# mpieva/network-aware-bwa

Measured on AMD Instinct MI355X. Metric: aligned reads/s to GRCh38 (100 bp SE), FM-index search (bwa_cal_sa_reg_gap), bit-exact vs CPU, higher is better.
Workload: dtype u32

## Files before the change

network-aware-bwa_amd/csrc/fm_index.hip:

```cpp
#include "nabwa_dev.hpp"
#include "launchers.hpp"

__device__ __forceinline__ uint32_t ref_base(const uint32_t *w, uint32_t j)
{
	const uint32_t *p = w + (size_t)(j >> 7) * 12 + 4;
	return p[(j & 127u) >> 4] >> ((~j & 15u) << 1) & 3u;
}

__global__ __launch_bounds__(256) void repack_kernel(const uint32_t *__restrict__ w, uint32_t seq_len,
													 uint32_t n_buckets, uint4 *__restrict__ out)
{
	const uint32_t b = blockIdx.x * 256u + threadIdx.x;
	if (b >= n_buckets) return;
	const uint32_t j0 = b * NABWA_INTV;
	uint32_t cnt[4] = {0, 0, 0, 0};
	if (j0 <= seq_len) {
		const uint32_t blk = j0 >> 7;
		const uint32_t *p = w + (size_t)blk * 12;
		cnt[0] = p[0]; cnt[1] = p[1]; cnt[2] = p[2]; cnt[3] = p[3];
		for (uint32_t j = blk << 7; j < j0; ++j) ++cnt[ref_base(w, j)];
	}
	uint64_t lo[3] = {0, 0, 0}, hi[3] = {0, 0, 0};
	for (uint32_t g = 0; g < 3; ++g) {
		for (uint32_t q = 0; q < 4; ++q) {
// ... 50 lines not shown
	k /= intv;
	out[idx] = steps + (k ? sa[k] : 0xffffffffu);
}

extern "C" void nabwa_launch_sa_lookup(const DevBwt *B, int n, const uint8_t *which, const uint32_t *k, uint32_t *out,
									   hipStream_t s)
{
	if (n <= 0) return;
	hipLaunchKernelGGL(sa_lookup_kernel, dim3((n + 255) / 256), dim3(256), 0, s, B[0], B[1], n, which, k, out);
}

__global__ __launch_bounds__(256) void occ4_kernel(DevBwt B, int n, const uint32_t *__restrict__ k, uint32_t *__restrict__ out)
{
	const int idx = blockIdx.x * 256 + threadIdx.x;
	if (idx >= n) return;
	const Occ4 o = nabwa_occ4(B, k[idx]);
	out[4 * idx] = o.c[0]; out[4 * idx + 1] = o.c[1]; out[4 * idx + 2] = o.c[2]; out[4 * idx + 3] = o.c[3];
}

extern "C" void nabwa_launch_occ4(const DevBwt *B, int n, const uint32_t *k, uint32_t *out, hipStream_t s)
{
	if (n <= 0) return;
	hipLaunchKernelGGL(occ4_kernel, dim3((n + 255) / 256), dim3(256), 0, s, *B, n, k, out);
}

__global__ __launch_bounds__(256) void kmer_level_kernel(DevBwt B, const uint2 *__restrict__ prev, uint2 *__restrict__ cur, uint64_t n_par)
{
	const uint64_t idx = (uint64_t)blockIdx.x * 256u + threadIdx.x;
	if (idx >= n_par) return;
	const uint2 par = prev ? prev[idx] : make_uint2(0u, B.seq_len);
	uint2 out[4];
#pragma unroll
	for (int c = 0; c < 4; ++c) out[c] = make_uint2(1u, 0u);
	if (par.x <= par.y) {
		Occ4 ck, cl;
		nabwa_occ4_pair(B, par.x - 1u, par.y, ck, cl);
#pragma unroll
		for (int c = 0; c < 4; ++c) {
			const uint32_t k = B.L2[c] + ck.c[c] + 1u, l = B.L2[c] + cl.c[c];
			if (k <= l) out[c] = make_uint2(k, l);
		}
	}
	uint4 *const dst = (uint4*)(cur + 4 * idx);
	dst[0] = make_uint4(out[0].x, out[0].y, out[1].x, out[1].y);
	dst[1] = make_uint4(out[2].x, out[2].y, out[3].x, out[3].y);
}

extern "C" void nabwa_launch_kmer_level(const DevBwt *B, const uint2 *prev, uint2 *cur, uint64_t n_cur, hipStream_t s)
{
	const uint64_t n_par = n_cur / 4;
	hipLaunchKernelGGL(kmer_level_kernel, dim3((unsigned int)((n_par + 255) / 256)), dim3(256), 0, s, *B, prev, cur, n_par);
}

__global__ __launch_bounds__(256) void sa_fill_kernel(DevBwt B, uint32_t *__restrict__ sa_full, uint32_t *__restrict__ isa,
												  uint8_t *__restrict__ text_bytes)
{
	const uint32_t j = blockIdx.x * 256u + threadIdx.x;
	if (j >= B.n_sa) return;
	uint32_t row = j * B.sa_intv, v = j ? B.sa[j] : B.seq_len;
	sa_full[row] = j ? v : 0xffffffffu;
	isa[v] = row;
	for (;;) {
		if (row == B.primary) break;
		const uint32_t kp = row - (row > B.primary ? 1u : 0u);
		const uint32_t b = kp / NABWA_INTV, r = kp - b * NABWA_INTV;
		const uint4 *p = B.bk + (size_t)b * 4;
		const uint4 q0 = p[0], q1 = p[1], q2 = p[2], q3 = p[3];
		const uint32_t c = nabwa_base_at(q1, q2, q3, r);
		const Occ4 o = nabwa_count4(q0, q1, q2, q3, r);
		v -= 1u;
		text_bytes[v] = (uint8_t)c;
		row = B.L2[c] + o.c[c];
		if (row % B.sa_intv == 0u) break;
		sa_full[row] = v; isa[v] = row;
	}
}

__global__ __launch_bounds__(256) void text_pack_kernel(const uint8_t *__restrict__ bytes, uint32_t n, uint32_t n_words, uint32_t *__restrict__ out)
{
	const uint32_t w = blockIdx.x * 256u + threadIdx.x;
	if (w >= n_words) return;
	uint32_t x = 0;
	for (uint32_t t = 0; t < 16u; ++t) { const uint64_t j = (uint64_t)w * 16u + t; if (j < n) x |= (uint32_t)(bytes[j] & 3u) << (2u * t); }
	out[w] = x;
}

extern "C" void nabwa_launch_sa_fill(const DevBwt *B, uint32_t *sa_full, uint32_t *isa, uint8_t *text_bytes, hipStream_t s)
{
	hipLaunchKernelGGL(sa_fill_kernel, dim3((B->n_sa + 255) / 256), dim3(256), 0, s, *B, sa_full, isa, text_bytes);
}
extern "C" void nabwa_launch_text_pack(const uint8_t *bytes, uint32_t n, uint32_t n_words, uint32_t *out, hipStream_t s)
{
	hipLaunchKernelGGL(text_pack_kernel, dim3((n_words + 255) / 256), dim3(256), 0, s, bytes, n, n_words, out);
}
```

network-aware-bwa_amd/csrc/fm_search.hip:

```cpp
#include "nabwa_dev.hpp"
#include "fm_search.hpp"
#include "launchers.hpp"

#define STATE_M 0
#define STATE_I 1
#define STATE_D 2
#define STATE_GROUP 3
#define GRP_EXT 0x100u
#define TXM 0xfffffffeu
#define KEYM 0xffffffffu
#define LVO(t_) ((size_t)((((uint64_t)1 << (2 * (t_))) - 4ull) / 3ull))
#ifndef NABWA_W_WAVES
#define NABWA_W_WAVES 5
#endif
#ifndef NABWA_WORK_CHUNK
#define NABWA_WORK_CHUNK 64u
#endif
#ifndef NABWA_RUN_MAX
#define NABWA_RUN_MAX 4
#endif

__device__ __forceinline__ uint32_t byte_of(uint64_t lo, uint64_t hi, uint32_t idx)
{
	asm volatile("" : "+v"(lo), "+v"(hi));
	const uint64_t h = (idx & 8u) ? hi : lo;
	return (uint32_t)(h >> ((idx & 7u) << 3)) & 0xffu;
}
#define WIN_SET(lo_, hi_, a_, b_, c_, d_) do { lo_ = (uint64_t)(b_) << 32 | (a_); hi_ = (uint64_t)(d_) << 32 | (c_); } while (0)

__device__ __forceinline__ void set_word(uint4 &q, uint32_t c, uint32_t v)
{
	q.x = c == 0 ? v : q.x; q.y = c == 1 ? v : q.y; q.z = c == 2 ? v : q.z; q.w = c == 3 ? v : q.w;
}

extern __shared__ uint16_t s_head[];

#ifndef NABWA_MIN_WAVES
#define NABWA_MIN_WAVES 4
#endif

template <bool COUNT>
__global__ __launch_bounds__(NABWA_SEARCH_BLOCK, NABWA_W_WAVES) void fm_width_kernel(const SearchParams P)
{
	const uint32_t lane = threadIdx.x & 63u;
	bool run = false, done = false;
	unsigned int w_next = 0, w_end = 0;
	uint32_t rid = 0, x = 0; int len = 0, phase = 0, wi = 0, n = 0, sbase = 0, nN = 0;
	uint32_t sq_off = 0;
#define WREC (P.wdata + (size_t)rid * P.wstride)
#define BX(f_) (x ? P.bwt[1].f_ : P.bwt[0].f_)
	bool tmode = false; uint32_t tp = 0, twtag = 0xffffffffu; uint2 twin = make_uint2(0u, 0u);
	const bool text_ok = (P.text_mode & 1) && P.bwt[0].sa_full && P.bwt[1].sa_full;
	uint32_t kk = 0, ll = 0, pw = 0; int bid = 0;
	uint32_t wkey = 0xffffffffu; bool tok = false; int tbase = 0;
	const int KT = (int)P.bwt[0].kmer_T, LW = (int)P.bwt[0].kmer_LW;
	auto rekey = [&](int from) {
		tok = false; tbase = from;
		if (!KT || !P.rd_pack || from + 4 >= n) return;
		const int PW = P.pack_stride / 2;
		const uint32_t *const pk = P.rd_pack + (size_t)rid * P.pack_stride + x * PW;
		if (pk[PW - 1]) return;
		const int q = sbase + from;
		const uint32_t w0 = pk[q >> 4], w1 = pk[(q >> 4) + 1], sh = ((uint32_t)q & 15u) << 1;
		const uint32_t k16 = sh ? (w0 << sh) | (w1 >> (32u - sh)) : w0;
		wkey = k16 >> (2 * (16 - KT)); tok = true;
	};
	uint4 wacc = make_uint4(0, 0, 0, 0); uint64_t blo = 0, bhi = 0, slo = 0, shi = 0; int stag = -1;
	unsigned long long touches = 0;

	for (;;) {
		unsigned long long need = __ballot(!run && !done);
		if (P.w_sync && __ballot(run) != 0ull) need = 0ull;
		if (need) {
			if (w_next == w_end) {
				unsigned int base = 0;
				if (lane == 0) base = atomicAdd(P.work_counter + WC_WIDTH, (unsigned int)NABWA_WORK_CHUNK);
				w_next = __builtin_amdgcn_readfirstlane(base); w_end = w_next + NABWA_WORK_CHUNK;
			}
			const unsigned int rank = (unsigned int)__popcll(need & ((1ull << lane) - 1ull)), avail = w_end - w_next;
			const unsigned int base = w_next;
			w_next += min((unsigned int)__popcll(need), avail);
			if (!run && !done && rank < avail) {
				const unsigned int idx = base + rank;
				if (idx < 2u * (unsigned int)P.n) {
					rid = P.ids ? (uint32_t)P.ids[idx >> 1] : idx >> 1; x = idx & 1u;
					const int64_t o = P.poff[rid];
					len = P.rd_len[rid];
					sq_off = (uint32_t)o;
					nN = 0; stag = -1;
					if (P.w_skip_clean && P.n_aln[rid] == 0) {  }
					else if (len > 0) {
						run = true; phase = 0; wi = 0; n = len; sbase = 0; tmode = false;
						if (KT) { wkey = P.rd_key[6 * (size_t)rid + 2 + x]; tok = wkey != 0xffffffffu; }
						tbase = 0;
						kk = 0; ll = BX(seq_len); bid = 0; pw = 0; blo = bhi = 0;
					} else { if (x == 0u) P.rd_nN[rid] = 0; if (P.rd_cls) P.rd_cls[2 * (size_t)rid + x] = 0; }
				} else done = true;
			}
		}
		if (__ballot(!done) == 0ull) break;
		auto out_pos = [&](int p, bool last) {
			uint8_t *const rec = WREC;
			if (last) ++bid;
			const uint32_t wv = last ? 0u : ll - kk + 1u;
			const uint32_t bv = (uint32_t)(bid > 127 ? 127 : bid) | ((p > 0 && wv == pw) ? 128u : 0u);
			set_word(wacc, (uint32_t)p & 3u, wv);
			{ const uint64_t sh = (uint64_t)bv << (((uint32_t)p & 7u) << 3); if (p & 8) bhi |= sh; else blo |= sh; }
			pw = wv;
			if (phase == 0 && ((p & 3) == 3 || last)) *(uint4*)((uint32_t*)rec + x * P.WL + (p & ~3)) = wacc;
			if ((p & 15) == 15 || last) {
				*(uint4*)(rec + (phase ? P.woff_sbid + x * P.SLB : P.woff_bid + x * P.WLB) + (p & ~15)) =
					make_uint4((uint32_t)blo, (uint32_t)(blo >> 32), (uint32_t)bhi, (uint32_t)(bhi >> 32));
				blo = bhi = 0;
			}
		};
		bool bulk = run && phase == 0 && tmode && (wi & 15) == 0 && wi + 16 < n && tp >= 16u && pw == 1u;
		if (bulk) {
			if ((wi >> 4) != stag) { const uint4 q = *(const uint4*)((x ? P.rseq : P.seq) + sq_off + wi); WIN_SET(slo, shi, q.x, q.y, q.z, q.w); stag = wi >> 4; }
			const uint32_t w0 = (tp - 16u) >> 4;
			const uint32_t *const txt = BX(text);
			const uint32_t t0 = txt[w0], t1 = txt[w0 + 1u];
			auto squeeze = [](uint64_t v) -> uint32_t {
				uint64_t y = v & 0x0303030303030303ull;
				y = (y | y >> 6) & 0x000F000F000F000Full; y = (y | y >> 12) & 0x000000FF000000FFull; y = (y | y >> 24) & 0xFFFFull;
				return (uint32_t)y;
			};
			const bool clean = ((slo | shi) & 0xFCFCFCFCFCFCFCFCull) == 0ull;
			const uint32_t rd = squeeze(slo) | squeeze(shi) << 16;
			const uint32_t tx = (uint32_t)(((uint64_t)t1 << 32 | t0) >> (((tp - 16u) & 15u) << 1));
			uint32_t rv = __brev(tx); rv = (rv >> 1 & 0x55555555u) | (rv & 0x55555555u) << 1;
			bulk = clean && rv == rd;
			if (bulk) {
				uint8_t *const rec = WREC;
				uint32_t *const wp = (uint32_t*)rec + x * P.WL + wi;
#pragma unroll
				for (int u = 0; u < 4; ++u) *(uint4*)(wp + 4 * u) = make_uint4(1u, 1u, 1u, 1u);
				const uint32_t b4 = ((uint32_t)(bid > 127 ? 127 : bid) | 128u) * 0x01010101u;
				*(uint4*)(rec + P.woff_bid + x * P.WLB + wi) = make_uint4(b4, b4, b4, b4);
				tp -= 16u; wi += 16;
			}
		}
		if (bulk) {  }
		else if (run && tok && wi - tbase + 4 <= LW && wi + 4 < n) {
			uint2 tv[4];
			const uint2 *const lo = BX(kmer_lo);
#pragma unroll
			for (int u = 0; u < 4; ++u) {
				const int t = wi - tbase + u + 1;
				tv[u] = (lo + (size_t)((((uint64_t)1 << (2 * t)) - 4ull) / 3ull))[wkey >> (2 * (KT - t))];
			}
#pragma unroll
			for (int u = 0; u < 4; ++u) {
				kk = tv[u].x; ll = tv[u].y;
				const bool dead = kk > ll;
				if (dead) { kk = 0; ll = BX(seq_len); ++bid; }
				out_pos(wi, false);
				++wi;
				if (dead) { rekey(wi); break; }
			}
		} else if (run) {
			const int pos = sbase + wi;
			if ((pos >> 4) != stag) { const uint4 q = *(const uint4*)((x ? P.rseq : P.seq) + sq_off + (pos & ~15)); WIN_SET(slo, shi, q.x, q.y, q.z, q.w); stag = pos >> 4; }
			const int cc = (int)byte_of(slo, shi, (uint32_t)pos & 15u);
			uint4 qa[4], qb[4]; uint32_t rk = 0, rl = 0, sav = 0; bool kval = false, two = false;
#pragma unroll
			for (int u = 0; u < 4; ++u) { qa[u] = make_uint4(0, 0, 0, 0); qb[u] = make_uint4(0, 0, 0, 0); }
			const bool q = cc < 4 && !tmode;
			if (q) {
				const uint32_t primary = BX(primary), kq = kk - 1u, lq = ll;
				const uint32_t kp = kq - (kq >= primary ? 1u : 0u), lp = lq - (lq >= primary ? 1u : 0u);
				const uint32_t bl = lp / NABWA_INTV; rl = lp - bl * NABWA_INTV;
				kval = kq != 0xffffffffu;
				const uint32_t bkk = kval ? kp / NABWA_INTV : bl; rk = kp - bkk * NABWA_INTV;
				two = bkk != bl;
				const uint4 *const bkt = BX(bk);
				const uint4 *pl = bkt + (size_t)bl * 4, *pk = bkt + (size_t)bkk * 4;
#pragma unroll
				for (int u = 0; u < 4; ++u) qa[u] = pl[u];
				if (two) {
#pragma unroll
					for (int u = 0; u < 4; ++u) qb[u] = pk[u];
				}
				if (COUNT) touches += ref_touches(x ? P.bwt[1] : P.bwt[0], kq, lq, false);
				if (text_ok && kk == ll) sav = BX(sa_full)[kk];
			}
			if (tmode && tp > 0u && ((tp - 1u) >> 5) != twtag) {
				twtag = (tp - 1u) >> 5;
				twin = *(const uint2*)(BX(text) + 2 * (size_t)twtag);
			}
			if (tmode) {
				bool ok = cc < 4 && tp > 0u;
				if (ok) {
					const uint32_t t = tp - 1u, wd = (t & 16u) ? twin.y : twin.x;
					ok = (wd >> ((t & 15u) << 1) & 3u) == (uint32_t)cc;
					if (ok) tp = t;
				}
				if (cc > 3 && x == 0u && phase == 0) ++nN;
				if (!ok) { tmode = false; kk = 0; ll = BX(seq_len); ++bid; rekey(wi + 1); }
			} else {
				const bool was_one = text_ok && cc < 4 && kk == ll;
				if (cc < 4) {
					Occ4 ck, cl;
// ... 733 lines not shown
```

network-aware-bwa_amd/csrc/fm_search.hpp:

```cpp
#pragma once
#include <stdint.h>
#include "nabwa_dev.hpp"
#include "search_slots.hpp"

#define NABWA_SEARCH_BLOCK 256
#define NABWA_ST_OK        0
#define NABWA_ST_OVERFLOW  1
#define NABWA_ST_WIDE      2
#define NABWA_ST_POOL      3
#define NABWA_ST_HITCAP    4
#define NABWA_ST_GROWN     5

struct SearchParams {
	DevBwt bwt[2];
	const uint8_t *seq, *rseq;
	const int64_t *poff;
	const int32_t *rd_len;
	const uint8_t *rd_maxdiff, *rd_maxgapo;
	const int32_t *ids;
	const int32_t *res_slot;
	int n;
	int s_mm, s_gapo, s_gape, mode, indel_end_skip, max_del_occ, max_entries, max_gape, max_seed_diff, seed_len, max_top2;
	uint8_t *wdata;
	size_t wstride;
	uint32_t woff_bid, woff_sbid;
	uint32_t WL, WLB, SLB;
	int text_mode;
	const uint32_t *rd_key;
	uint8_t *rd_nN;
	uint8_t *scratch;
	size_t lane_stride;
	uint32_t cap, NS;
	int32_t *n_aln, *max_ent;
	uint8_t *status;
	uint4 *aln;
	int aln_cap;
	unsigned int *work_counter;
	uint32_t trip_budget;
	uint32_t trip_budget_hard;
	int sync_refill;
	const uint32_t *rd_pack; int pack_stride;
	int w_sync;
	int w_skip_clean;
	uint8_t *rd_cls;
	const unsigned int *n_sync;
	unsigned long long *touch_counter;
	const uint32_t *ixtab;
	int sure0;
	unsigned long long *s0_stats;
};

#define NABWA_IXTAB_STRIDE 24
#define NABWA_IXTAB_WORDS  48
#define IX_BK 0
#define IX_KMER 2
#define IX_KMER_LO 4
#define IX_TEXT 6
#define IX_ISA 8
#define IX_SA_FULL 10
#define IX_PRIMARY 12
#define IX_SEQ_LEN 13
#define IX_L2 13
static inline void nabwa_ixtab_fill(uint32_t *tab, const DevBwt *bwt )
{
	for (int q = 0; q < 2; ++q) {
		uint32_t *o = tab + NABWA_IXTAB_STRIDE * q;
		const uint64_t p[6] = { (uint64_t)(uintptr_t)bwt[q].bk, (uint64_t)(uintptr_t)bwt[q].kmer, (uint64_t)(uintptr_t)bwt[q].kmer_lo,
								(uint64_t)(uintptr_t)bwt[q].text, (uint64_t)(uintptr_t)bwt[q].isa, (uint64_t)(uintptr_t)bwt[q].sa_full };
		for (int f = 0; f < 6; ++f) { o[2 * f] = (uint32_t)p[f]; o[2 * f + 1] = (uint32_t)(p[f] >> 32); }
		o[IX_PRIMARY] = bwt[q].primary; o[IX_SEQ_LEN] = bwt[q].seq_len; o[IX_L2 + 1] = bwt[q].L2[1]; o[IX_L2 + 2] = bwt[q].L2[2]; o[IX_L2 + 3] = bwt[q].L2[3];
		for (int f = 17; f < NABWA_IXTAB_STRIDE; ++f) o[f] = 0;
	}
}
```

network-aware-bwa_amd/csrc/launchers.hpp:

```cpp
#pragma once
#include <hip/hip_runtime.h>
#include "fm_deep.hpp"

extern "C" {
void nabwa_launch_repack(const uint32_t *w, uint32_t seq_len, uint32_t n_buckets, uint4 *out, hipStream_t s);
void nabwa_launch_kmer_level(const DevBwt *B, const uint2 *prev, uint2 *cur, uint64_t n_cur, hipStream_t s);
void nabwa_launch_sa_fill(const DevBwt *B, uint32_t *sa_full, uint32_t *isa, uint8_t *text_bytes, hipStream_t s);
void nabwa_launch_text_pack(const uint8_t *bytes, uint32_t n, uint32_t n_words, uint32_t *out, hipStream_t s);
void nabwa_launch_sa_lookup(const DevBwt *B, int n, const uint8_t *which, const uint32_t *k, uint32_t *out, hipStream_t s);
void nabwa_launch_occ4(const DevBwt *B, int n, const uint32_t *k, uint32_t *out, hipStream_t s);
void nabwa_launch_fm_search(const SearchParams *P, int n_blocks, hipStream_t s);
void nabwa_launch_fm_width(const SearchParams *P, int n_blocks, hipStream_t s);
int nabwa_width_occupancy(void);
int nabwa_search_occupancy(int ns);
void nabwa_launch_checksum(int n, const int32_t *map, const uint32_t *cent, const uint8_t *arena, const int32_t *n_aln, const uint4 *aln, int aln_cap, const uint8_t *status,
						   const int32_t *wide_idx, const uint4 *aln2, int aln_cap2, const uint4 *const *grown,
						   unsigned long long *sum, unsigned long long *rows, hipStream_t s);
void nabwa_launch_collect(int n, const uint8_t *status, int32_t *ids, unsigned int *count, int which, hipStream_t s);
void nabwa_launch_collect_keyed(int n, const uint8_t *status, int32_t *ids, unsigned int *count, int which,
								const uint8_t *cls, const uint8_t *md, int max_key, const int32_t *n_aln, int aln_cap, hipStream_t s);
void nabwa_launch_assign_slots(int n2, const int32_t *ids, int32_t *wide_idx, hipStream_t s);
void nabwa_launch_scatter_grown(int n2, const int32_t *ids, const int32_t *n_aln3, const int32_t *max_ent3, const uint8_t *status3,
								 int32_t *n_aln, int32_t *max_ent, uint8_t *status, int32_t *wide_idx, const uint4 *block, size_t cap3,
								 const uint4 **grown, int slot0, hipStream_t s);
void nabwa_launch_scatter_wide(int n2, const int32_t *ids, const int32_t *n_aln2, const int32_t *max_ent2,
							   const uint8_t *status2, int32_t *n_aln, int32_t *max_ent, uint8_t *status,
							   int32_t *wide_idx, hipStream_t s);
void nabwa_launch_gather(int n, const int32_t *map, const uint32_t *cent, const uint8_t *arena, const int32_t *n_aln, const uint32_t *row_off, const uint4 *aln, int aln_cap,
						 const uint8_t *status, const int32_t *wide_idx, const uint4 *aln2, int aln_cap2,
						 const uint4 *const *grown, uint4 *out, hipStream_t s);
void nabwa_launch_partition(int n, const uint8_t *cls, int32_t *ids, unsigned int *cnt, hipStream_t s);
void nabwa_launch_padded_len(int n, const int64_t *off, int64_t *plen, hipStream_t s);
void nabwa_launch_pad_reads(int n, const uint8_t *seq, const uint8_t *rseq, const int64_t *off, const int64_t *poff,
							uint8_t *pseq, uint8_t *prseq, int32_t *rd_len, uint32_t *rd_key, int T, int seed_len, uint32_t *rd_pack, int pack_stride,
							const uint8_t *md_tab, const uint8_t *mg_tab, uint8_t *rd_md, uint8_t *rd_mg, hipStream_t s);
void nabwa_launch_dedup_hash(int n, const uint8_t *seq, const uint8_t *rseq, const int64_t *off, uint64_t mask, uint64_t *keys, uint32_t *ids, hipStream_t s);
void nabwa_launch_dedup_heads(int n, const uint64_t *keys, uint32_t *head, hipStream_t s);
void nabwa_launch_dedup_verify(int n, const uint8_t *seq, const uint8_t *rseq, const int64_t *off, const uint32_t *ids, const uint32_t *head,
							   int32_t *rep, uint32_t *flag, unsigned int *n_coll, hipStream_t s);
void nabwa_launch_dedup_map(int n, const int32_t *rep, const uint32_t *inner, const int64_t *off, int32_t *map, int64_t *clen, unsigned int *stat, hipStream_t s);
void nabwa_launch_dedup_compact(int n, const uint8_t *seq, const uint8_t *rseq, const int64_t *off, const int32_t *rep, const uint32_t *inner,
								const int64_t *coff, uint8_t *cseq, uint8_t *crseq, hipStream_t s);
void nabwa_launch_dedup_expand(int n, const int32_t *map, const int32_t *n_aln, const int32_t *max_ent, const uint32_t *cent, const uint8_t *arena,
							   int32_t *n_aln_out, int32_t *max_ent_out, hipStream_t s);
void nabwa_launch_dcache_lookup(int n, const uint8_t *seq, const uint8_t *rseq, const int64_t *off, const uint64_t *hash, const uint8_t *md_tab, const uint8_t *mg_tab,
								const unsigned long long *slots, uint32_t n_slots, uint64_t mask, const uint8_t *arena, uint32_t *found, uint32_t *flag, hipStream_t s);
void nabwa_launch_dcache_map(int n, const uint32_t *found, const uint32_t *inner, const int64_t *off, int32_t *rep, int32_t *newidx, int64_t *clen, uint32_t *cent,
							 unsigned int *stat, hipStream_t s);
void nabwa_launch_dcache_remap(int n, const int32_t *old, const int32_t *newidx, int32_t *map, hipStream_t s);
void nabwa_launch_dcache_insert(int n, const uint8_t *seq, const uint8_t *rseq, const int64_t *poff, const int32_t *len, const uint8_t *rd_md, const uint8_t *rd_mg,
								const uint8_t *status, const int32_t *n_aln, const int32_t *max_ent, const uint4 *aln, int aln_cap, const int32_t *wide_idx,
								const uint4 *aln2, int aln_cap2, const uint4 *const *grown, int row_cap, uint64_t mask,
								unsigned long long *slots, uint32_t n_slots, uint8_t *arena, uint64_t arena_bytes, unsigned long long *ctr, hipStream_t s);
void nabwa_launch_fm_deep(const DeepParams *P, int n_waves, hipStream_t s);
int nabwa_deep_occupancy(int ns, int lds_rd);
void nabwa_launch_bgzf_deflate(const uint8_t *in, int64_t n, int n_slices, uint8_t *stage, uint32_t *sizes, hipStream_t s);
void nabwa_launch_bgzf_deflate_dyn(const uint8_t *in, int64_t n, int n_slices, uint8_t *stage, uint32_t *sizes, hipStream_t s);
void nabwa_launch_bgzf_pack(const uint8_t *stage, const uint32_t *sizes, int n_slices, uint8_t *packed, int64_t *total, hipStream_t s);
struct BgzfInBlk;
// ... 12 lines not shown
```

network-aware-bwa_amd/csrc/nabwa_batch.hip:

```cpp
#include <hip/hip_runtime.h>
#include <hipcub/hipcub.hpp>
#include <stdio.h>
#include <stdlib.h>
#include <string.h>
#include <memory>
#include <mutex>
#include <vector>
#include "../../include/nabwa.h"
#include "nabwa_batch.hpp"
#include "dedup_cache_body.hpp"
#include "host_util.hpp"

static void layout(SearchParams &P, uint32_t cap, int max_len, int seed_len, uint32_t NS)
{
	P.WL = align_up((uint32_t)max_len + 1, 16);
	P.WLB = P.WL + 16;
	P.SLB = align_up((uint32_t)(max_len > seed_len ? seed_len : 0) + 1, 16) + 16;
	P.woff_bid = 2 * P.WL * 4;
	P.woff_sbid = P.woff_bid + 2 * P.WLB;
	P.wstride = align_up(P.woff_sbid + 2 * P.SLB, 64);
	P.cap = cap; P.NS = NS;
	P.lane_stride = align_up((size_t)cap * 16, 64);
}

// ... 223 lines not shown
	if ((uint64_t)pnb >= (1ull << 32)) return nabwa_fail(NABWA_EINVAL, "batch holds 4 Gi padded bases or more: split it (lane state keeps a 32-bit read offset)");
	auto read_buffers = [&](int n) -> int {
		HIP_CHECK(b->d_seq.get(ix, pnb)); HIP_CHECK(b->d_rseq.get(ix, pnb));
		HIP_CHECK(b->d_poff.get(ix, (size_t)(n + 1) * 8)); HIP_CHECK(b->d_len.get(ix, (size_t)(n ? n : 1) * 4));
		HIP_CHECK(b->d_md.get(ix, n ? n : 1)); HIP_CHECK(b->d_mg.get(ix, n ? n : 1)); HIP_CHECK(b->d_key.get(ix, (size_t)(n ? n : 1) * 24));
		b->pack_stride = 2 * ((max_len + 15) / 16 + 2);
		HIP_CHECK(b->d_pack.get(ix, (size_t)(n ? n : 1) * b->pack_stride * 4));
		HIP_CHECK(b->d_cls.get(ix, (size_t)(n ? n : 1) * 2)); HIP_CHECK(b->d_perm.get(ix, (size_t)(n ? n : 1) * 4)); HIP_CHECK(b->d_ncls.get(ix, NCLS_WORDS * sizeof(unsigned int)));
		return NABWA_OK;
	};
	const bool dedup = dedup_bits >= 0 && n_given > 0;
	if (!dedup) if (int r = read_buffers(n_given)) return r;
	if (n_given == 0) { HIP_CHECK(hipMemset(b->d_poff, 0, 8)); return NABWA_OK; }
	PoolBuf<uint8_t> raw_s, raw_r, d_tab; PoolBuf<int64_t> raw_off, plen; PoolBuf<void> d_tmp; size_t tmp_bytes = 0;
	StreamDrain drain{ b->stream };
	HIP_CHECK(raw_s.get(ix, nb)); HIP_CHECK(raw_r.get(ix, nb)); HIP_CHECK(raw_off.get(ix, (size_t)(n_given + 1) * 8));
	const UploadJob jobs[3] = { { raw_s, seq, (size_t)off[n_given] }, { raw_r, rseq, (size_t)off[n_given] }, { raw_off, off, (size_t)(n_given + 1) * 8 } };
	const double tu0 = now_s();
	HIP_CHECK(staged_upload(ix, jobs, 3));
	if (timing) fprintf(stderr, "[nabwa] upload of %.2f GB: %.3f s (%.3f s into batch_create)\n", 2e-9 * (double)off[n_given], now_s() - tu0, tu0 - tc0);
	if (dedup) {
		if (int r = dedup_reads(b, dedup_bits, raw_s, raw_r, raw_off, nb, timing)) return r;
		if (b->cache) if (int r = cache_lookup(b, s, raw_s, raw_r, raw_off, nb, timing)) return r;
		if (int r = read_buffers(b->n)) return r;
	}
	const int n = b->n;
	HIP_CHECK(plen.get(ix, (size_t)(n + 1) * 8));
	nabwa_launch_padded_len(n, raw_off, plen, b->stream);
	HIP_CHECK(hipcub::DeviceScan::ExclusiveSum(nullptr, tmp_bytes, plen.p, b->d_poff.p, n + 1, b->stream));
	HIP_CHECK(d_tmp.get(ix, tmp_bytes ? tmp_bytes : 16));
	HIP_CHECK(hipcub::DeviceScan::ExclusiveSum(d_tmp.p, tmp_bytes, plen.p, b->d_poff.p, n + 1, b->stream));
	HIP_CHECK(d_tab.get(ix, 2 * (size_t)(max_len + 1)));
	HIP_CHECK(hipMemcpyAsync(d_tab, s.md_tab.data(), max_len + 1, hipMemcpyHostToDevice, b->stream));
	HIP_CHECK(hipMemcpyAsync(d_tab + max_len + 1, s.mg_tab.data(), max_len + 1, hipMemcpyHostToDevice, b->stream));
	nabwa_launch_pad_reads(n, raw_s, raw_r, raw_off, b->d_poff, b->d_seq, b->d_rseq, b->d_len, b->d_key,
						   ix->bwt[0].kmer_T == ix->bwt[1].kmer_T ? (int)ix->bwt[0].kmer_T : 0, b->opt.seed_len, b->d_pack, b->pack_stride,
						   d_tab, d_tab + max_len + 1, b->d_md, b->d_mg, b->stream);
	HIP_CHECK(hipStreamSynchronize(b->stream));
	if (timing) fprintf(stderr, "[nabwa] re-layout kernel done %.3f s into batch_create\n", now_s() - tc0);
	HIP_CHECK(raw_s.release()); HIP_CHECK(raw_r.release()); HIP_CHECK(raw_off.release());
	HIP_CHECK(plen.release()); HIP_CHECK(d_tmp.release()); HIP_CHECK(d_tab.release());
	return NABWA_OK;
}

static int working_buffers(nabwa_batch *b, const BatchShape &s)
{
	nabwa_index *ix = b->ix;
	const nabwa_gap_opt_t *opt = &b->opt;
	const int n = b->n, max_len = s.max_len;
	SearchParams &P = b->P;
	memset(&P, 0, sizeof(P));
	P.bwt[0] = ix->bwt[0]; P.bwt[1] = ix->bwt[1];
	{
		uint32_t tab[NABWA_IXTAB_WORDS];
		nabwa_ixtab_fill(tab, ix->bwt);
		HIP_CHECK(b->d_ixtab.get(ix, sizeof tab));
		HIP_CHECK(hipMemcpy(b->d_ixtab, tab, sizeof tab, hipMemcpyHostToDevice));
		P.ixtab = b->d_ixtab;
	}
	P.seq = b->d_seq; P.rseq = b->d_rseq; P.poff = b->d_poff; P.rd_len = b->d_len; P.rd_maxdiff = b->d_md; P.rd_maxgapo = b->d_mg; P.rd_key = b->d_key; P.rd_pack = b->d_pack; P.pack_stride = b->pack_stride;
	P.text_mode = env_int("NABWA_TEXT_KERNELS", 7);
	if (ix->bwt[0].kmer_T != ix->bwt[1].kmer_T) P.bwt[0].kmer_T = P.bwt[1].kmer_T = 0;
	P.ids = 0; P.n = n;
	P.s_mm = opt->s_mm; P.s_gapo = opt->s_gapo; P.s_gape = opt->s_gape; P.mode = opt->mode;
	P.indel_end_skip = opt->indel_end_skip; P.max_del_occ = opt->max_del_occ; P.max_entries = opt->max_entries;
	P.max_gape = opt->max_gape; P.max_seed_diff = opt->max_seed_diff; P.seed_len = opt->seed_len; P.max_top2 = opt->max_top2;
	int cap1 = env_int("NABWA_CAP1", 4096);
	if (cap1 < 16) cap1 = 16;
	if (cap1 > 65534) cap1 = 65534;
	layout(P, (uint32_t)cap1, max_len, opt->seed_len, s.deep_only ? 1u : s.NS1);
	P.aln_cap = env_int("NABWA_ALNCAP1", 16);
	P.sync_refill = env_int("NABWA_SYNC_REFILL", 0);
	P.trip_budget = (uint32_t)env_int("NABWA_TRIP_BUDGET", max_len > opt->seed_len ? 2000 : 300);
	P.trip_budget_hard = (uint32_t)env_int("NABWA_TRIP_BUDGET_HARD", max_len > opt->seed_len ? 200 : (int)P.trip_budget);
	if (getenv("NABWA_TRIP_BUDGET") && !getenv("NABWA_TRIP_BUDGET_HARD")) P.trip_budget_hard = P.trip_budget;
	b->class_sort = env_int("NABWA_CLASS_SORT", 1);
	P.sure0 = env_int("NABWA_SURE0", 3);
	if (P.sure0 < 0) P.sure0 = 0;
	if (P.sure0 > 3) P.sure0 = 3;
	if (env_int("NABWA_SURE0_STATS", 0)) {
		HIP_CHECK(b->d_s0stats.get(ix, S0S_WORDS * sizeof(unsigned long long)));
		HIP_CHECK(hipMemset(b->d_s0stats, 0, S0S_WORDS * sizeof(unsigned long long)));
		P.s0_stats = b->d_s0stats;
	}
	{
		P.w_sync = (n > 0 && s.min_len == max_len) ? env_int("NABWA_W_SYNC", 1) : 0;
	}
	if (P.aln_cap < 1) P.aln_cap = 1;

	hipDeviceProp_t prop;
	HIP_CHECK(hipGetDeviceProperties(&prop, ix->device));
	int occ = nabwa_search_occupancy(s.deep_only ? 1 : (int)s.NS1);
	if (occ < 1) occ = 1;
	const int occ_env = env_int("NABWA_BLOCKS_PER_CU", 0);
	if (occ_env > 0) occ = occ_env;
	long blocks = (long)prop.multiProcessorCount * occ;
	const long need = ((long)n + NABWA_SEARCH_BLOCK - 1) / NABWA_SEARCH_BLOCK;
	if (blocks > need) blocks = need;
	if (blocks < 1) blocks = 1;
	b->n_blocks = (int)blocks;
	if (getenv("NABWA_TIMING")) fprintf(stderr, "[nabwa] search kernel: %u score levels, %d blocks per CU (LDS %zu B per block), %ld blocks\n", s.NS1, occ,
										(size_t)s.NS1 * NABWA_SEARCH_BLOCK * 2 + NABWA_SEARCH_BLOCK * 80, blocks);
	HIP_CHECK(b->d_scratch.get(ix, (size_t)blocks * NABWA_SEARCH_BLOCK * P.lane_stride));
	int occw = nabwa_width_occupancy(); if (occw < 1) occw = 1;
	long blocks_w = (long)prop.multiProcessorCount * occw;
	if (blocks_w > 2 * need) blocks_w = 2 * need;
	if (blocks_w < 1) blocks_w = 1;
	b->n_blocks_w = (int)blocks_w;
	HIP_CHECK(b->d_wdata.get(ix, (size_t)(n ? n : 1) * P.wstride));
	HIP_CHECK(b->d_nN.get(ix, n ? n : 1));
	P.wdata = b->d_wdata; P.rd_nN = b->d_nN;
	const size_t n1 = n ? n : 1;
	HIP_CHECK(b->d_naln.get(ix, n1 * 4)); HIP_CHECK(b->d_maxent.get(ix, n1 * 4)); HIP_CHECK(b->d_wide_idx.get(ix, n1 * 4));
	HIP_CHECK(b->d_status.get(ix, n1)); HIP_CHECK(b->d_aln.get(ix, n1 * (size_t)P.aln_cap * 16));
// ... 379 lines not shown
```

network-aware-bwa_amd/csrc/nabwa_index.hip:

```cpp
#include <hip/hip_runtime.h>
#include <stdio.h>
#include <stdlib.h>
#include <string.h>
#include <memory>
#include <string>
#include <vector>
#include "../../include/nabwa.h"
#include "launchers.hpp"
#include "dedup_cache_body.hpp"
#include "nabwa_internal.hpp"
#include "dev_pool.hpp"
#include "finish_gpu.hpp"

static int build_one(nabwa_index *ix, int t_, const uint32_t *words, uint64_t n_words, bool on_device,
					 const uint32_t *sa_words, uint64_t n_sa_words)
{
	uint32_t hdr[5];
	if (n_words < 5) return nabwa_fail(NABWA_EIO, "bwt array too short");
	if (on_device) HIP_CHECK(hipMemcpy(hdr, words, 20, hipMemcpyDeviceToHost)); else memcpy(hdr, words, 20);
	DevBwt &B = ix->bwt[t_];
	memset(&B, 0, sizeof(B));
	B.primary = hdr[0]; B.L2[0] = 0; B.L2[1] = hdr[1]; B.L2[2] = hdr[2]; B.L2[3] = hdr[3]; B.seq_len = hdr[4];
	if (B.seq_len > 0xffffffdfu) return nabwa_fail(NABWA_EINVAL, "seq_len above 0xffffffdf: the reference's SA count wraps (bwtio.c:175)");
	const uint64_t expect = ((uint64_t)B.seq_len + 15) / 16 + (((uint64_t)B.seq_len + 127) / 128 + 1) * 4;
	if (n_words - 5 < expect) return nabwa_fail(NABWA_EIO, "bwt array shorter than its seq_len implies");
	B.n_buckets = (uint32_t)(((uint64_t)B.seq_len + NABWA_INTV - 1) / NABWA_INTV);
	DevBuf raw;
	const uint32_t *src = words + 5;
	if (!on_device) {
		if (int r = raw.get((n_words - 5) * 4)) return r;
		HIP_CHECK(hipMemcpy(raw.p, words + 5, (n_words - 5) * 4, hipMemcpyHostToDevice));
		src = raw.as<uint32_t>();
	}
	HIP_CHECK(hipMalloc(&ix->bk[t_], (size_t)B.n_buckets * 64));
	nabwa_launch_repack(src, B.seq_len, B.n_buckets, ix->bk[t_], 0);
	HIP_CHECK(hipGetLastError());
	HIP_CHECK(hipDeviceSynchronize());
	HIP_CHECK(raw.release());
	B.bk = ix->bk[t_];
	ix->bytes += (uint64_t)B.n_buckets * 64;
	{
		int T = 0;
		for (uint64_t x = B.seq_len; x >= 4; x >>= 2) ++T;
		T += 1;
		const char *e = getenv("NABWA_KMER_T");
		if (e) T = atoi(e);
		if (T > 16) T = 16;
		size_t free_b = 0, total_b = 0;
		HIP_CHECK(hipMemGetInfo(&free_b, &total_b));
		auto table_entries = [](int t) { size_t x = 0; for (int u = 1; u <= t; ++u) x += (size_t)1 << (2 * u); return x; };
		if (ix->kmer_T_pick < 0) {
			while (T > 12 && 2 * table_entries(T) * 8 > free_b / 5 * 3) --T;
			ix->kmer_T_pick = T;
		} else {
			T = ix->kmer_T_pick;
			if (T >= 1 && table_entries(T) * 8 > free_b / 10 * 9) {
				fprintf(stderr, "[nabwa] WARNING: no device memory for the second interval table of depth %d (%zu MB free): the search runs WITHOUT interval tables "
								"(several times slower); free device memory or set NABWA_KMER_T lower\n", T, free_b >> 20);
				T = 0;
			}
		}
		if (T >= 1) {
			const size_t lo_n = table_entries(T);
			HIP_CHECK(hipMalloc(&ix->kmer[t_], lo_n * 8));
			uint2 *prev = 0, *cur = ix->kmer[t_];
			for (int t = 1; t <= T; ++t) {
				nabwa_launch_kmer_level(&B, prev, cur, (uint64_t)1 << (2 * t), 0);
				prev = cur; cur += (size_t)1 << (2 * t);
			}
			HIP_CHECK(hipGetLastError());
			HIP_CHECK(hipDeviceSynchronize());
			ix->bytes += lo_n * 8;
			B.kmer = prev; B.kmer_T = (uint32_t)T; B.kmer_lo = ix->kmer[t_]; B.kmer_LW = (uint32_t)T;
		}
	}
	if (sa_words) {
		uint32_t sh[7];
		if (n_sa_words < 7) return nabwa_fail(NABWA_EIO, "sa array too short");
		if (on_device) HIP_CHECK(hipMemcpy(sh, sa_words, 28, hipMemcpyDeviceToHost)); else memcpy(sh, sa_words, 28);
		if (sh[0] != B.primary || sh[6] != B.seq_len) return nabwa_fail(NABWA_EIO, "SA-BWT inconsistency");
		B.sa_intv = sh[5];
		if (B.sa_intv < 1 || (uint64_t)B.seq_len + B.sa_intv > 0xffffffffull)
			return nabwa_fail(NABWA_EINVAL, "seq_len + sa_intv above 0xffffffff: the reference's SA count wraps (bwtio.c:175)");
		B.n_sa = (uint32_t)(((uint64_t)B.seq_len + B.sa_intv) / B.sa_intv);
		if (n_sa_words - 7 < (uint64_t)B.n_sa - 1) return nabwa_fail(NABWA_EIO, "sa array shorter than n_sa");
		HIP_CHECK(hipMalloc(&ix->sa[t_], (size_t)B.n_sa * 4));
		HIP_CHECK(hipMemset(ix->sa[t_], 0xff, 4));
		HIP_CHECK(hipMemcpy(ix->sa[t_] + 1, sa_words + 7, (size_t)(B.n_sa - 1) * 4,
						 on_device ? hipMemcpyDeviceToDevice : hipMemcpyHostToDevice));
		B.sa = ix->sa[t_];
		ix->bytes += (uint64_t)B.n_sa * 4;
		const char *tm = getenv("NABWA_TEXT_MODE");
		if (!(tm && atoi(tm) == 0)) {
			const size_t rows = (size_t)B.seq_len + 1, words = ((size_t)B.seq_len + 15) / 16 + 4;
			DevBuf tb;
			HIP_CHECK(hipMalloc(&ix->sa_full[t_], rows * 4)); HIP_CHECK(hipMalloc(&ix->isa[t_], rows * 4));
			HIP_CHECK(hipMalloc(&ix->text[t_], words * 4)); if (int r = tb.get(rows)) return r;
			nabwa_launch_sa_fill(&B, ix->sa_full[t_], ix->isa[t_], tb.as<uint8_t>(), 0);
			nabwa_launch_text_pack(tb.as<uint8_t>(), B.seq_len, (uint32_t)words, ix->text[t_], 0);
			HIP_CHECK(hipGetLastError());
			HIP_CHECK(hipDeviceSynchronize());
			HIP_CHECK(tb.release());
			B.sa_full = ix->sa_full[t_]; B.isa = ix->isa[t_]; B.text = ix->text[t_];
			ix->bytes += rows * 8 + words * 4;
		}
	}
	return NABWA_OK;
}

extern "C" int nabwa_index_from_arrays(int device, int is_device, const uint32_t *bwt0, uint64_t nw0,
									   const uint32_t *bwt1, uint64_t nw1, const uint32_t *sa0, uint64_t ns0,
									   const uint32_t *sa1, uint64_t ns1, nabwa_index_t **out)
{
	if (!out || !bwt0 || !bwt1) return nabwa_fail(NABWA_EINVAL, "null argument");
	if (nabwa_device_count() <= device) return nabwa_fail(NABWA_ENODEV, "no such HIP device");
	HIP_CHECK(hipSetDevice(device));
	nabwa_index *ix = new nabwa_index();
	ix->pool = pool_create();
	ix->device = device;
	int r = build_one(ix, 0, bwt0, nw0, is_device != 0, sa0, ns0);
	if (r == NABWA_OK) r = build_one(ix, 1, bwt1, nw1, is_device != 0, sa1, ns1);
	if (r != NABWA_OK) { nabwa_index_destroy(ix); return r; }
	*out = ix;
	return NABWA_OK;
// ... 6 lines not shown
	fseek(f, 0, SEEK_END); long n = ftell(f); fseek(f, 0, SEEK_SET);
	v.resize((n + 3) / 4);
	bool ok = fread(v.data(), 1, n, f) == (size_t)n;
	fclose(f);
	return ok;
}

extern "C" int nabwa_index_load(const char *prefix, int device, int with_sa, int with_pac, nabwa_index_t **out)
{
	if (!prefix || !out) return nabwa_fail(NABWA_EINVAL, "null argument");
	std::vector<uint32_t> b0, b1, s0, s1;
	std::string p(prefix);
	if (!slurp(p + ".bwt", b0)) return nabwa_fail(NABWA_EIO, "cannot read %s.bwt", prefix);
	if (!slurp(p + ".rbwt", b1)) return nabwa_fail(NABWA_EIO, "cannot read %s.rbwt", prefix);
	if (with_sa) {
		if (!slurp(p + ".sa", s0)) return nabwa_fail(NABWA_EIO, "cannot read %s.sa", prefix);
		if (!slurp(p + ".rsa", s1)) return nabwa_fail(NABWA_EIO, "cannot read %s.rsa", prefix);
	}
	int r = nabwa_index_from_arrays(device, 0, b0.data(), b0.size(), b1.data(), b1.size(),
									with_sa ? s0.data() : 0, s0.size(), with_sa ? s1.data() : 0, s1.size(), out);
	if (r == NABWA_OK && with_pac) {
		r = nabwa_index_attach_reference(*out, prefix);
		if (r != NABWA_OK) { nabwa_index_destroy(*out); *out = 0; }
	}
	return r;
}

extern "C" void nabwa_index_destroy(nabwa_index_t *ix)
{
	if (!ix) return;
	(void)hipSetDevice(ix->device);
	for (int t = 0; t < 2; ++t) { if (ix->bk[t]) (void)hipFree(ix->bk[t]); if (ix->sa[t]) (void)hipFree(ix->sa[t]); if (ix->kmer[t]) (void)hipFree(ix->kmer[t]); if (ix->kmer_top[t]) (void)hipFree(ix->kmer_top[t]);
		if (ix->sa_full[t]) (void)hipFree(ix->sa_full[t]); if (ix->isa[t]) (void)hipFree(ix->isa[t]); if (ix->text[t]) (void)hipFree(ix->text[t]); }
	nabwa_finish_drop_reference(ix);
	if (nabwa_dedup_cache *c = ix->dcache) {
		if (c->d_slots) (void)pool_free(ix, c->d_slots);
		if (c->d_arena) (void)pool_free(ix, c->d_arena);
		if (c->d_ctr) (void)pool_free(ix, c->d_ctr);
		delete c;
	}
	pool_destroy(ix->pool);
	if (ix->d_ntpac) (void)hipFree(ix->d_ntpac);
	delete ix->ref_nt;
	delete ix->ref;
	delete ix;
}

extern "C" int nabwa_index_export(const nabwa_index_t *ix, int which, int what, uint64_t first, uint64_t n, uint32_t *out)
{
	if (!ix || !out || which < 0 || which > 1) return nabwa_fail(NABWA_EINVAL, "bad argument");
	HIP_CHECK(hipSetDevice(ix->device));
	const DevBwt &B = ix->bwt[which];
	if (what == 4) { out[0] = B.kmer_T; return NABWA_OK; }
	if (what == 3) {
		if (!B.kmer || first + n > (1ull << (2 * B.kmer_T))) return nabwa_fail(NABWA_EINVAL, "no interval table / out of range");
		HIP_CHECK(hipMemcpy(out, B.kmer + first, n * 8, hipMemcpyDeviceToHost));
		return NABWA_OK;
	}
	if (!B.sa_full) return nabwa_fail(NABWA_EINVAL, "index has no text-mode companions (no SA given, or NABWA_TEXT_MODE=0)");
	if (what == 0 || what == 1) {
		if (first + n > (uint64_t)B.seq_len + 1) return nabwa_fail(NABWA_EINVAL, "out of range");
		HIP_CHECK(hipMemcpy(out, (what ? B.isa : B.sa_full) + first, n * 4, hipMemcpyDeviceToHost));
		return NABWA_OK;
	}
	if (what == 2) {
		if (first + n > (uint64_t)B.seq_len) return nabwa_fail(NABWA_EINVAL, "out of range");
		const uint64_t w0 = first / 16, w1 = (first + n + 15) / 16;
		std::vector<uint32_t> w(w1 - w0);
		HIP_CHECK(hipMemcpy(w.data(), B.text + w0, (w1 - w0) * 4, hipMemcpyDeviceToHost));
		for (uint64_t j = 0; j < n; ++j) { const uint64_t p = first + j; out[j] = w[p / 16 - w0] >> (2 * (p & 15)) & 3u; }
		return NABWA_OK;
	}
	return nabwa_fail(NABWA_EINVAL, "unknown part");
}

extern "C" uint32_t nabwa_index_seq_len(const nabwa_index_t *ix, int which) { return ix->bwt[which & 1].seq_len; }
extern "C" uint64_t nabwa_index_device_bytes(const nabwa_index_t *ix) { return ix->bytes; }


int nabwa_dcache_get(nabwa_index *ix, long mib, nabwa_dedup_cache **out)
{
	std::lock_guard<std::mutex> lk(ix->dcache_mu);
	if (ix->dcache) { *out = ix->dcache; return NABWA_OK; }
	uint64_t budget = (uint64_t)mib << 20;
	size_t free_b = 0, total_b = 0;
	HIP_CHECK(hipMemGetInfo(&free_b, &total_b));
	{ std::lock_guard<std::mutex> pk(ix->pool->mu); free_b += ix->pool->idle_bytes; }
	if (budget > free_b) {
		char why[160]; snprintf(why, sizeof why, "NABWA_DEDUP_CACHE=%ld: more MiB than the device has free (%zu)", mib, free_b >> 20);
		return nabwa_fail(NABWA_EINVAL, "%s", why);
	}
	if (budget > (65535ull << 20)) budget = 65535ull << 20;
	uint32_t n_slots = 1024;
	while ((uint64_t)n_slots * 2 * 8 <= budget / 8 && n_slots < (1u << 30)) n_slots *= 2;
	const uint64_t ctr_bytes = DC_WORDS * sizeof(unsigned long long);
	const uint64_t arena_bytes = (budget - (uint64_t)n_slots * 8 - ctr_bytes) & ~(uint64_t)15;
	std::unique_ptr<nabwa_dedup_cache> c(new nabwa_dedup_cache());
	hipError_t e = pool_malloc(ix, (void**)&c->d_slots, (size_t)n_slots * 8);
	if (e == hipSuccess) e = pool_malloc(ix, (void**)&c->d_arena, arena_bytes);
	if (e == hipSuccess) e = pool_malloc(ix, (void**)&c->d_ctr, ctr_bytes);
	if (e == hipSuccess) e = hipMemset(c->d_slots, 0, (size_t)n_slots * 8);
	if (e == hipSuccess) e = hipMemset(c->d_ctr, 0, ctr_bytes);
	if (e != hipSuccess) {
		if (c->d_slots) (void)pool_free(ix, c->d_slots);
		if (c->d_arena) (void)pool_free(ix, c->d_arena);
		if (c->d_ctr) (void)pool_free(ix, c->d_ctr);
// ... 78 lines not shown
```

network-aware-bwa_amd/csrc/nabwa_internal.hpp:

```cpp
#pragma once
#include <stdint.h>
#include <stdio.h>
#include <mutex>
#include <string>
#include <vector>
#include "../../include/nabwa.h"
#include "fm_search.hpp"
#include "host_util.hpp"

struct nabwa_ann { int64_t offset; int32_t len, n_ambs; std::string name; };
struct nabwa_hole { int64_t offset; int32_t len; char amb; };

struct nabwa_reference {
	int64_t l_pac; uint32_t seed;
	std::vector<nabwa_ann> anns;
	std::vector<nabwa_hole> holes;
	std::vector<uint8_t> pac;
};

struct nabwa_dedup_cache {
	std::mutex mu;
	unsigned long long *d_slots = nullptr; uint32_t n_slots = 0;
	uint8_t *d_arena = nullptr; uint64_t arena_bytes = 0;
	unsigned long long *d_ctr = nullptr;
	uint64_t reserved = 0;
	bool has_sig = false; uint64_t sig = 0;
	int pins = 0;
	uint64_t used = 0, entries = 0;
	uint64_t lookups = 0, served = 0, flushes = 0, bypasses = 0;
};

struct nabwa_index {
	int device = 0;
	DevBwt bwt[2] = {};
	uint4 *bk[2] = {};
	uint32_t *sa[2] = {};
	uint32_t *sa_full[2] = {}, *isa[2] = {}, *text[2] = {};
	uint2 *kmer[2] = {}, *kmer_top[2] = {};
	uint64_t bytes = 0;
	int kmer_T_pick = -1;
	nabwa_reference *ref = nullptr;
	nabwa_reference *ref_nt = nullptr;
	uint8_t *d_ntpac = nullptr;
	uint64_t ntpac_bytes = 0;
	struct nabwa_dev_pool *pool = nullptr;
	std::mutex fin_mu;
	uint8_t *d_pac = nullptr; uint64_t pac_bytes = 0;
	void *d_holes[2] = {}; uint64_t holes_bytes[2] = {}; int n_holes_dev[2] = {};
	bool fin_ready[2] = {};
	std::mutex dcache_mu;
	nabwa_dedup_cache *dcache = nullptr;
};

int nabwa_dcache_get(nabwa_index *ix, long mib, nabwa_dedup_cache **out);
int nabwa_dcache_reset(nabwa_index *ix, nabwa_dedup_cache *c);

static inline int nabwa_hip_fail(hipError_t e, const char *expr, const char *file, int line)
{
	char b[512]; snprintf(b, sizeof b, "%s failed: %s (%s:%d)", expr, hipGetErrorString(e), file, line);
	return nabwa_fail(NABWA_ENODEV, "%s", b);
}
#define HIP_CHECK(x) do { const hipError_t e_ = (x); if (e_ != hipSuccess) return nabwa_hip_fail(e_, #x, __FILE__, __LINE__); } while (0)

int nabwa_se_posn_strided(nabwa_index_t *ix, const nabwa_gap_opt_t *opt, int n, const int64_t *off, const int32_t *full_len,
						  const int32_t *n_aln, const nabwa_aln1_t *aln, const uint8_t *n_occ_v, uint64_t *rng48, void *out_base, size_t stride);
int nabwa_se_refine_strided(nabwa_index_t *ix, int n, const int64_t *off, const uint8_t *seq, const uint8_t *rseq, void *out_base, size_t stride);
int nabwa_reference_read(const char *prefix, nabwa_reference **out);
int nabwa_cs2nt_records(nabwa_index_t *ix, void *base, size_t stride, int n, const int64_t *off, const uint8_t *seq, const uint8_t *rseq,
						const uint8_t *qual, uint8_t *nt_seq, uint8_t *nt_rseq, uint8_t *nt_qual, double *times);
void nabwa_poscache_register(nabwa_poscache_t *cache, int max_occ, int n, const int *first, const int32_t *n_aln, const int64_t *row0,
							 const nabwa_aln1_t *rows, const nabwa_pe_t *res);
```

Before: 103.3 million.

## Derive two k-mer levels per quad load using primary-row correction

In the k-mer table walk, the kernel now loads the four child intervals (two uint4s) of a level and derives the parent interval's size from their sum plus a correction for the BWT primary row. It also selects the next-level interval from those same loads, so four levels take two gathers instead of four. To support this, index build runs a small kernel that records, per level, which k-mer interval contains the primary row, and stores those values in the ixtab device table and in shared memory. The per-read pack-sentinel check is hoisted to read start. The risk is bit-exactness: the derived interval is (1,size) rather than the true (k,l), which only holds if downstream code uses just the interval width at those steps.

```diff
diff --git a/network-aware-bwa_amd/csrc/fm_index.hip b/network-aware-bwa_amd/csrc/fm_index.hip
--- a/network-aware-bwa_amd/csrc/fm_index.hip
+++ b/network-aware-bwa_amd/csrc/fm_index.hip
@@ -126,6 +126,24 @@
 	hipLaunchKernelGGL(kmer_level_kernel, dim3((unsigned int)((n_par + 255) / 256)), dim3(256), 0, s, *B, prev, cur, n_par);
 }
 
+__global__ __launch_bounds__(256) void kmer_primary_kernel(const uint2 *__restrict__ lv, uint64_t n_par, uint32_t primary, uint32_t *__restrict__ out)
+{
+	const uint64_t idx = (uint64_t)blockIdx.x * 256u + threadIdx.x;
+	if (idx >= n_par) return;
+	const uint4 *const src = (const uint4*)(lv + 4 * idx);
+	const uint4 a = src[0], b = src[1];
+	const uint2 e[4] = { make_uint2(a.x, a.y), make_uint2(a.z, a.w), make_uint2(b.x, b.y), make_uint2(b.z, b.w) };
+#pragma unroll
+	for (int c = 0; c < 4; ++c)
+		if (e[c].x <= e[c].y && e[c].x <= primary && primary <= e[c].y) *out = (uint32_t)(4 * idx + c);
+}
+
+extern "C" void nabwa_launch_kmer_primary(const uint2 *lv, uint64_t n_keys, uint32_t primary, uint32_t *out, hipStream_t s)
+{
+	const uint64_t n_par = n_keys / 4;
+	hipLaunchKernelGGL(kmer_primary_kernel, dim3((unsigned int)((n_par + 255) / 256)), dim3(256), 0, s, lv, n_par, primary, out);
+}
+
 __global__ __launch_bounds__(256) void sa_fill_kernel(DevBwt B, uint32_t *__restrict__ sa_full, uint32_t *__restrict__ isa,
 												  uint8_t *__restrict__ text_bytes)
 {
diff --git a/network-aware-bwa_amd/csrc/fm_search.hip b/network-aware-bwa_amd/csrc/fm_search.hip
--- a/network-aware-bwa_amd/csrc/fm_search.hip
+++ b/network-aware-bwa_amd/csrc/fm_search.hip
@@ -54,12 +54,16 @@
 	uint32_t kk = 0, ll = 0, pw = 0; int bid = 0;
 	uint32_t wkey = 0xffffffffu; bool tok = false; int tbase = 0;
 	const int KT = (int)P.bwt[0].kmer_T, LW = (int)P.bwt[0].kmer_LW;
+	__shared__ uint32_t s_pk[2 * NABWA_PK_LEVELS];
+	const bool quads = (P.text_mode & TM_W_QUADS) && P.ixtab;
+	if (threadIdx.x < 2 * NABWA_PK_LEVELS) s_pk[threadIdx.x] = quads ? P.ixtab[NABWA_IXTAB_WORDS + threadIdx.x] : 0xffffffffu;
+	__syncthreads();
+	bool nflag = true;
 	auto rekey = [&](int from) {
 		tok = false; tbase = from;
-		if (!KT || !P.rd_pack || from + 4 >= n) return;
+		if (nflag || from + 4 >= n) return;
 		const int PW = P.pack_stride / 2;
 		const uint32_t *const pk = P.rd_pack + (size_t)rid * P.pack_stride + x * PW;
-		if (pk[PW - 1]) return;
 		const int q = sbase + from;
 		const uint32_t w0 = pk[q >> 4], w1 = pk[(q >> 4) + 1], sh = ((uint32_t)q & 15u) << 1;
 		const uint32_t k16 = sh ? (w0 << sh) | (w1 >> (32u - sh)) : w0;
@@ -92,6 +96,7 @@
 					else if (len > 0) {
 						run = true; phase = 0; wi = 0; n = len; sbase = 0; tmode = false;
 						if (KT) { wkey = P.rd_key[6 * (size_t)rid + 2 + x]; tok = wkey != 0xffffffffu; }
+						nflag = !KT || !P.rd_pack || P.rd_pack[(size_t)rid * P.pack_stride + (x + 1u) * (uint32_t)(P.pack_stride / 2) - 1u] != 0u;
 						tbase = 0;
 						kk = 0; ll = BX(seq_len); bid = 0; pw = 0; blo = bhi = 0;
 					} else { if (x == 0u) P.rd_nN[rid] = 0; if (P.rd_cls) P.rd_cls[2 * (size_t)rid + x] = 0; }
@@ -144,10 +149,30 @@
 		else if (run && tok && wi - tbase + 4 <= LW && wi + 4 < n) {
 			uint2 tv[4];
 			const uint2 *const lo = BX(kmer_lo);
-#pragma unroll
-			for (int u = 0; u < 4; ++u) {
-				const int t = wi - tbase + u + 1;
-				tv[u] = (lo + (size_t)((((uint64_t)1 << (2 * t)) - 4ull) / 3ull))[wkey >> (2 * (KT - t))];
+			const int t1 = wi - tbase + 1;
+			if (quads) {
+				uint4 qd[2][2];
+#pragma unroll
+				for (int h = 0; h < 2; ++h) {
+					const int t = t1 + 2 * h;
+					const uint4 *const p = (const uint4*)(lo + LVO(t + 1) + 4 * (size_t)(wkey >> (2 * (KT - t))));
+					qd[h][0] = p[0]; qd[h][1] = p[1];
+				}
+#pragma unroll
+				for (int h = 0; h < 2; ++h) {
+					const int t = t1 + 2 * h;
+					const uint32_t ch = wkey >> (2 * (KT - t - 1)), c = ch & 3u;
+					const uint4 a = qd[h][0], b = qd[h][1];
+					const uint32_t sum = (a.y - a.x) + (a.w - a.z) + (b.y - b.x) + (b.w - b.z) + 4u + ((ch >> 2) == s_pk[x * NABWA_PK_LEVELS + t] ? 1u : 0u);
+					tv[2 * h] = make_uint2(1u, sum);
+					tv[2 * h + 1] = c == 0u ? make_uint2(a.x, a.y) : (c == 1u ? make_uint2(a.z, a.w) : (c == 2u ? make_uint2(b.x, b.y) : make_uint2(b.z, b.w)));
+				}
+			} else {
+#pragma unroll
+				for (int u = 0; u < 4; ++u) {
+					const int t = t1 + u;
+					tv[u] = (lo + LVO(t))[wkey >> (2 * (KT - t))];
+				}
 			}
 #pragma unroll
 			for (int u = 0; u < 4; ++u) {
diff --git a/network-aware-bwa_amd/csrc/fm_search.hpp b/network-aware-bwa_amd/csrc/fm_search.hpp
--- a/network-aware-bwa_amd/csrc/fm_search.hpp
+++ b/network-aware-bwa_amd/csrc/fm_search.hpp
@@ -10,6 +10,8 @@
 #define NABWA_ST_POOL      3
 #define NABWA_ST_HITCAP    4
 #define NABWA_ST_GROWN     5
+
+#define TM_W_QUADS 8
 
 struct SearchParams {
 	DevBwt bwt[2];
@@ -52,6 +54,8 @@
 
 #define NABWA_IXTAB_STRIDE 24
 #define NABWA_IXTAB_WORDS  48
+#define NABWA_PK_LEVELS    17
+#define NABWA_IXTAB_ALL    (NABWA_IXTAB_WORDS + 2 * NABWA_PK_LEVELS)
 #define IX_BK 0
 #define IX_KMER 2
 #define IX_KMER_LO 4
diff --git a/network-aware-bwa_amd/csrc/launchers.hpp b/network-aware-bwa_amd/csrc/launchers.hpp
--- a/network-aware-bwa_amd/csrc/launchers.hpp
+++ b/network-aware-bwa_amd/csrc/launchers.hpp
@@ -5,6 +5,7 @@
 extern "C" {
 void nabwa_launch_repack(const uint32_t *w, uint32_t seq_len, uint32_t n_buckets, uint4 *out, hipStream_t s);
 void nabwa_launch_kmer_level(const DevBwt *B, const uint2 *prev, uint2 *cur, uint64_t n_cur, hipStream_t s);
+void nabwa_launch_kmer_primary(const uint2 *lv, uint64_t n_keys, uint32_t primary, uint32_t *out, hipStream_t s);
 void nabwa_launch_sa_fill(const DevBwt *B, uint32_t *sa_full, uint32_t *isa, uint8_t *text_bytes, hipStream_t s);
 void nabwa_launch_text_pack(const uint8_t *bytes, uint32_t n, uint32_t n_words, uint32_t *out, hipStream_t s);
 void nabwa_launch_sa_lookup(const DevBwt *B, int n, const uint8_t *which, const uint32_t *k, uint32_t *out, hipStream_t s);
diff --git a/network-aware-bwa_amd/csrc/nabwa_batch.hip b/network-aware-bwa_amd/csrc/nabwa_batch.hip
--- a/network-aware-bwa_amd/csrc/nabwa_batch.hip
+++ b/network-aware-bwa_amd/csrc/nabwa_batch.hip
@@ -299,14 +299,16 @@
 	memset(&P, 0, sizeof(P));
 	P.bwt[0] = ix->bwt[0]; P.bwt[1] = ix->bwt[1];
 	{
-		uint32_t tab[NABWA_IXTAB_WORDS];
+		uint32_t tab[NABWA_IXTAB_ALL];
 		nabwa_ixtab_fill(tab, ix->bwt);
+		memcpy(tab + NABWA_IXTAB_WORDS, ix->kmer_pk, sizeof ix->kmer_pk);
 		HIP_CHECK(b->d_ixtab.get(ix, sizeof tab));
 		HIP_CHECK(hipMemcpy(b->d_ixtab, tab, sizeof tab, hipMemcpyHostToDevice));
 		P.ixtab = b->d_ixtab;
 	}
 	P.seq = b->d_seq; P.rseq = b->d_rseq; P.poff = b->d_poff; P.rd_len = b->d_len; P.rd_maxdiff = b->d_md; P.rd_maxgapo = b->d_mg; P.rd_key = b->d_key; P.rd_pack = b->d_pack; P.pack_stride = b->pack_stride;
-	P.text_mode = env_int("NABWA_TEXT_KERNELS", 7);
+	P.text_mode = env_int("NABWA_TEXT_KERNELS", 7) & 7;
+	if (env_int("NABWA_W_QUADS", 1)) P.text_mode |= TM_W_QUADS;
 	if (ix->bwt[0].kmer_T != ix->bwt[1].kmer_T) P.bwt[0].kmer_T = P.bwt[1].kmer_T = 0;
 	P.ids = 0; P.n = n;
 	P.s_mm = opt->s_mm; P.s_gapo = opt->s_gapo; P.s_gape = opt->s_gape; P.mode = opt->mode;
diff --git a/network-aware-bwa_amd/csrc/nabwa_index.hip b/network-aware-bwa_amd/csrc/nabwa_index.hip
--- a/network-aware-bwa_amd/csrc/nabwa_index.hip
+++ b/network-aware-bwa_amd/csrc/nabwa_index.hip
@@ -20,6 +20,7 @@
 	if (on_device) HIP_CHECK(hipMemcpy(hdr, words, 20, hipMemcpyDeviceToHost)); else memcpy(hdr, words, 20);
 	DevBwt &B = ix->bwt[t_];
 	memset(&B, 0, sizeof(B));
+	memset(ix->kmer_pk[t_], 0xff, sizeof ix->kmer_pk[t_]);
 	B.primary = hdr[0]; B.L2[0] = 0; B.L2[1] = hdr[1]; B.L2[2] = hdr[2]; B.L2[3] = hdr[3]; B.seq_len = hdr[4];
 	if (B.seq_len > 0xffffffdfu) return nabwa_fail(NABWA_EINVAL, "seq_len above 0xffffffdf: the reference's SA count wraps (bwtio.c:175)");
 	const uint64_t expect = ((uint64_t)B.seq_len + 15) / 16 + (((uint64_t)B.seq_len + 127) / 128 + 1) * 4;
@@ -68,8 +69,15 @@
 				nabwa_launch_kmer_level(&B, prev, cur, (uint64_t)1 << (2 * t), 0);
 				prev = cur; cur += (size_t)1 << (2 * t);
 			}
+			DevBuf pk;
+			if (int r = pk.get(sizeof ix->kmer_pk[t_])) return r;
+			HIP_CHECK(hipMemsetAsync(pk.p, 0xff, sizeof ix->kmer_pk[t_], 0));
+			for (int t = 1; t <= T; ++t)
+				nabwa_launch_kmer_primary(ix->kmer[t_] + table_entries(t - 1), (uint64_t)1 << (2 * t), B.primary, pk.as<uint32_t>() + t, 0);
 			HIP_CHECK(hipGetLastError());
+			HIP_CHECK(hipMemcpy(ix->kmer_pk[t_], pk.p, sizeof ix->kmer_pk[t_], hipMemcpyDeviceToHost));
 			HIP_CHECK(hipDeviceSynchronize());
+			HIP_CHECK(pk.release());
 			ix->bytes += lo_n * 8;
 			B.kmer = prev; B.kmer_T = (uint32_t)T; B.kmer_lo = ix->kmer[t_]; B.kmer_LW = (uint32_t)T;
 		}
@@ -182,6 +190,11 @@
 	HIP_CHECK(hipSetDevice(ix->device));
 	const DevBwt &B = ix->bwt[which];
 	if (what == 4) { out[0] = B.kmer_T; return NABWA_OK; }
+	if (what == 5) {
+		if (first + n > NABWA_PK_LEVELS) return nabwa_fail(NABWA_EINVAL, "out of range");
+		memcpy(out, ix->kmer_pk[which] + first, n * 4);
+		return NABWA_OK;
+	}
 	if (what == 3) {
 		if (!B.kmer || first + n > (1ull << (2 * B.kmer_T))) return nabwa_fail(NABWA_EINVAL, "no interval table / out of range");
 		HIP_CHECK(hipMemcpy(out, B.kmer + first, n * 8, hipMemcpyDeviceToHost));
diff --git a/network-aware-bwa_amd/csrc/nabwa_internal.hpp b/network-aware-bwa_amd/csrc/nabwa_internal.hpp
--- a/network-aware-bwa_amd/csrc/nabwa_internal.hpp
+++ b/network-aware-bwa_amd/csrc/nabwa_internal.hpp
@@ -39,6 +39,7 @@
 	uint2 *kmer[2] = {}, *kmer_top[2] = {};
 	uint64_t bytes = 0;
 	int kmer_T_pick = -1;
+	uint32_t kmer_pk[2][NABWA_PK_LEVELS] = {};
 	nabwa_reference *ref = nullptr;
 	nabwa_reference *ref_nt = nullptr;
 	uint8_t *d_ntpac = nullptr;
```

Measured after the change: 111.2 million, median of 6. +7.7%, better.
